# charliezhang/ringpop

Hardware: AMD Instinct MI355X
Metric: gossip rounds/sec (member-updates/s) at 65,536 sim nodes, 1/2/4/8 GPUs (higher is better)
Workload: dtype u64

## Files before the change

### include/ringpop_hip.h

```cpp
#ifndef RINGPOP_HIP_H
#define RINGPOP_HIP_H

#include <stddef.h>
#include <stdint.h>

#ifdef __cplusplus
extern "C" {
#endif

#define RP_OK 0
#define RP_ERR_INVALID (-1)
#define RP_ERR_HIP (-2)
#define RP_ERR_NOMEM (-3)
#define RP_ERR_UNSUPPORTED (-4)
#define RP_ERR_CAPACITY (-5)
#define RP_ERR_STATE (-6)

const char *rp_last_error(void);
int rp_abi_version(void);
int rp_set_device(int device);

int rp_device_malloc(size_t bytes, void **out);
int rp_device_free(void *ptr);
int rp_device_memcpy(void *dst, const void *src, size_t bytes, int kind);
// ... 54 lines not shown
typedef struct rp_sim rp_sim;
typedef struct {
    uint32_t n;
    uint32_t churn_k;
    uint64_t seed;
    uint64_t arena_entries;
    uint32_t snapshot_slots;
    uint32_t origin_slots;
    uint32_t seen_window;
    uint32_t replica_hash_shift;
    uint32_t compact_mul;
    uint32_t compact_add;
    uint32_t prefix_min;
    uint32_t ck_lane_min;
    uint32_t issue_wave;
} rp_sim_config;

typedef struct {
    uint64_t evaluated;
    uint64_t applied;
    uint64_t full_syncs;
    uint64_t messages;
    uint64_t waves;
    uint64_t pings;
    uint64_t converged;
} rp_round_stats;

int rp_sim_create(const rp_sim_config *cfg, rp_sim **out);
int rp_sim_destroy(rp_sim *sim);

// ... 158 lines not shown
```

### ringpop_amd/_lib.py

```python
import ctypes
import os

_HERE = os.path.dirname(os.path.abspath(__file__))
LIB_PATH = os.environ.get("RINGPOP_HIP_LIB") or os.path.join(_HERE, "libringpop_hip.so")

RP_OK = 0
ERRORS = {-1: "invalid argument", -2: "HIP error", -3: "out of device memory", -4: "unsupported",
          -5: "capacity exceeded", -6: "kernel error"}


class RingpopError(RuntimeError):
    def __init__(self, code, msg):
        super().__init__(f"{ERRORS.get(code, code)}: {msg}")
        self.code = code


class SimConfig(ctypes.Structure):
    _fields_ = [("n", ctypes.c_uint32), ("churn_k", ctypes.c_uint32), ("seed", ctypes.c_uint64),
                ("arena_entries", ctypes.c_uint64), ("snapshot_slots", ctypes.c_uint32),
                ("origin_slots", ctypes.c_uint32), ("seen_window", ctypes.c_uint32), ("replica_hash_shift", ctypes.c_uint32),
                ("compact_mul", ctypes.c_uint32), ("compact_add", ctypes.c_uint32), ("prefix_min", ctypes.c_uint32),
                ("ck_lane_min", ctypes.c_uint32), ("issue_wave", ctypes.c_uint32)]


class RoundStats(ctypes.Structure):
    _fields_ = [(k, ctypes.c_uint64) for k in
                ("evaluated", "applied", "full_syncs", "messages", "waves", "pings", "converged")]

    def as_dict(self):
        return {k: int(getattr(self, k)) for k, _ in self._fields_}


class RouteStats(ctypes.Structure):
    _fields_ = [(k, ctypes.c_uint64) for k in
                ("requests", "local", "delivered", "checksums_differ", "unreachable", "entry_dead", "misrouted",
                 "reserved")]

# ... 193 lines not shown
```

### ringpop_amd/build.py

```python
import json
import os
import re
import subprocess
import sys
from concurrent.futures import ThreadPoolExecutor

HERE = os.path.dirname(os.path.abspath(__file__))
CSRC = os.path.join(HERE, "csrc")
OBJ = os.path.join(HERE, "build")
LIB = os.path.join(HERE, "libringpop_hip.so")
SOURCES = ["rp_capi.hip", "rp_ring.hip", "rp_sim.hip", "rp_traffic.hip", "rp_node.hip", "rp_calib.hip"]
_INCLUDE_RE = re.compile(r'^\s*#\s*include\s+"([^"]+)"', re.M)


def included_headers(sources=SOURCES, csrc=CSRC):
    seen, todo = set(), [os.path.join(csrc, s) for s in sources]
    while todo:
        path = todo.pop()
        with open(path) as f:
            text = f.read()
        for inc in _INCLUDE_RE.findall(text):
            h = os.path.normpath(os.path.join(os.path.dirname(path), inc))
            if h not in seen and os.path.exists(h):
                seen.add(h)
                todo.append(h)
    return sorted(os.path.relpath(h, csrc) for h in seen)


HEADERS = included_headers()
ARCH = os.environ.get("RINGPOP_OFFLOAD_ARCH", "gfx950")
HIPCC = os.environ.get("HIPCC", "/opt/rocm/bin/hipcc")
FLAGS = ["-O3", "-std=c++17", "-fPIC", "--offload-arch=" + ARCH, "-Wall", "-Wno-unused-function"]
VARIANTS = {
    "diag": ["-DRP_DIAG"],
    "alt": ["-DRP_ISSUE_UNR_P1=4", "-DRP_ISSUE_UNR=4", "-DRP_ISSUE_STASH=64", "-DRP_ISSUE_P2U=1", "-DRP_SETTLED_PF=0",
            "-DRP_KPT=2", "-DRP_P2_SPLIT=1", "-DRP_CKP_SHARED=0", "-DRP_CK_SIDE=0", "-DRP_SEEN_GROUP_LOG=1",
            "-DRP_COMPACT_MUL=2u", "-DRP_COMPACT_ADD=1024u", "-DRP_LOOKUP_DIR16=0", "-DRP_RING_INCR_MAX_POINTS=0",
            "-DRP_ISSUE_WAVE=0"],
}


def _mtime(p):
    return os.path.getmtime(p) if os.path.exists(p) else 0.0


def _stamp(flags):
    return json.dumps({"hipcc": os.path.realpath(HIPCC), "arch": ARCH, "flags": flags,
                       "sources": SOURCES}, sort_keys=True)


def variant_lib(variant):
    return LIB.replace(".so", "_" + variant + ".so")

# ... 46 lines not shown
```

### ringpop_amd/csrc/rp_sim.h

```cpp
#pragma once
#include <hip/hip_runtime.h>
#include <stdint.h>

#include <string>
#include <vector>

#include "rp_common.h"

namespace rp {

enum : uint32_t {
    SIMERR_ABSENT_MEMBER = 1u << 0,
    SIMERR_TIMERS_FULL = 1u << 1,
    SIMERR_ORIGIN_FULL = 1u << 2,
    SIMERR_ARENA_FULL = 1u << 3,
    SIMERR_SNAP_FULL = 1u << 4,
    SIMERR_RINGOPS = 1u << 5,
    SIMERR_PING_FAILED = 1u << 6,
    SIMERR_PREDICATE = 1u << 7,
    SIMERR_P2_LIST = 1u << 8,
    SIMERR_LIFECYCLE = 1u << 9,
};

enum : int32_t { RESP_NONE = 0, RESP_LIST = 1, RESP_EMPTY = 2, RESP_FS_PENDING = 3, RESP_FS = 4, RESP_ERR = 5,
                 RESP_LIST_RX = 6 };

struct Resp {
    int32_t kind;
    uint32_t from;
    uint64_t off;
    uint32_t len;
    uint32_t snap;
    uint32_t ping_status;
    uint32_t plen;
    uint32_t nesc;
    uint32_t eoff;
// ... 137 lines not shown
    uint32_t* rl_len;
    uint32_t* rl_nesc;
    uint64_t* rl_inc;
    uint64_t* rl_fp;
    uint32_t* rl_csum;
    uint2* tfifo;
    uint32_t* thead;
    uint32_t* ttail;
    uint32_t tcap;
    int32_t* churn_ids;
    unsigned long long* stats;
    unsigned long long* bstats;
    uint32_t bstride;
    uint32_t* err;
    uint32_t* conv;
};

enum {
    STAT_EVALUATED = 0, STAT_APPLIED, STAT_FULLSYNC, STAT_MESSAGES, STAT_WAVES, STAT_PINGS,
    STAT_EVAL_P2, STAT_APPLIED_P2, STAT_EVAL_P3, STAT_APPLIED_P3, STAT_SCANNED_P1, STAT_EMITTED_P1,
    STAT_SCANNED_P2, STAT_EMITTED_P2, STAT_WRITTEN_P1, STAT_WRITTEN_P2,
    STAT_TOUCHED, STAT_TOUCHED_P2,
    STAT_CK_VIEWS,
    STAT_COMPACT_ISSUE, STAT_COMPACT_APPLY,
    STAT_PREFIX_PACKS,
    STAT_SAME_VIEW,
    STAT_DIAG0, STAT_DIAG1, STAT_DIAG2, STAT_DIAG3, STAT_DIAG4, STAT_DIAG5,
    STAT_WAVE_ISSUES,
    STAT_NSTATS
};

__device__ inline bool cut(const SimDev& S, uint32_t a, uint32_t b) {
    return S.part_split > 0 && S.round >= S.part_start && S.round < S.part_end &&
           ((a < S.part_split) != (b < S.part_split));
}
__host__ __device__ inline uint8_t* gossip_off(const SimDev& S) { return S.dead + S.n; }
__host__ __device__ inline uint8_t* suspicion_off(const SimDev& S) { return S.dead + 2 * (size_t)S.n; }
__device__ inline bool unreachable(const SimDev& S, uint32_t from, uint32_t to) {
    return S.dead[to] || cut(S, from, to);
}

}
```

### ringpop_amd/csrc/rp_sim.hip

```cpp
#include <hip/hip_runtime.h>

#include <algorithm>
#include <chrono>
#include <condition_variable>
#include <memory>
#include <mutex>
#include <cmath>
#include <cstdio>
#include <cstdlib>
#include <cstring>
#include <numeric>
#include <stdexcept>
#include <string>
#include <type_traits>
#include <vector>

#include "rp_block.h"
#include "rp_checksum.h"
#include "rp_common.h"
#include "rp_sim.h"
#include "rp_traffic.h"
#include "rp_whash.h"

namespace rp {
// ... 2939 lines not shown
                r.kind = RESP_EMPTY;
            } else if (!csum_known) {
                atomicOr(S.err, SIMERR_PREDICATE);
                r.kind = RESP_EMPTY;
            } else {
                uint32_t k = atomicAdd(S.snap_count, 1u);
                if (k >= S.snap_cap) { atomicOr(S.err, SIMERR_SNAP_FULL); r.kind = RESP_EMPTY; }
                else {
                    r.kind = RESP_FS_PENDING; r.snap = k;
                    S.pend_slot[k] = csum_of_sender ? (slot | PEND_SND) : slot;
                    S.pend_csum[k] = req_csum;
                }
            }
        }
        S.resp[slot] = r;
        sh.u[7] = r.kind == RESP_FS_PENDING ? r.snap : NONE;
        stat_add(S, STAT_MESSAGES, 1ull);
    }
    lds_barrier();
    if (sh.u[7] != NONE) {
        uint64_t* dst = S.snaps + (size_t)sh.u[7] * n;
        const VEnt* srow = S.view + S.row(b);
        for (uint32_t a = threadIdx.x; a < n; a += BLOCK) dst[a] = srow[a].vs;
        const uint32_t M = S.mcount[b];
        uint32_t* dord = S.snap_ord + (size_t)sh.u[7] * n;
        const uint32_t* sord = S.order + S.row(b);
        for (uint32_t i = threadIdx.x; i < M; i += BLOCK) dord[i] = sord[i];
        if (threadIdx.x == 0) S.snap_m[sh.u[7]] = M;
    }
    lds_barrier();
// ... 19 lines not shown
        const uint32_t M = S.snap_m[r.snap];
        auto src = [&](uint32_t i) {
            Change c;
            c.addr = ord[i];
            c.origin = B;
            c.vs = snap[c.addr];
            return c;
        };
        wg_apply<JOIN, PRE>(S, x, src, M, M, now, weight, phase, sh, pre);
    }
}

#ifndef RP_P2_SPLIT
#define RP_P2_SPLIT 2
#endif
constexpr uint32_t P2_SPLIT = RP_P2_SPLIT;
constexpr uint32_t P2_DEAD = 0x80000000u;
__host__ __device__ inline uint32_t p2_grid(uint32_t nl, uint32_t n, uint32_t k) {
    const uint32_t b = n / (k + 1);
    return b < nl ? (b ? b : 1u) : nl;
}
constexpr uint64_t P2_RX = 1ull << 63;
__global__ void __launch_bounds__(256) k_p2_lists(SimDev S, uint32_t* lists, uint32_t* lens, uint64_t* msgs) {
    __shared__ uint32_t wbase[P2_SPLIT + 1][4], bbase[P2_SPLIT + 1];
    const uint32_t i = blockIdx.x * blockDim.x + threadIdx.x;
    const uint32_t b = S.lo + i;
    const uint32_t c = i < S.nl ? S.g_base[b + 1] - S.g_base[b] : 0u;
    const uint64_t below = (1ull << lane_id()) - 1ull;
    const int w = threadIdx.x >> 6;
    uint64_t m[P2_SPLIT + 1];
// ... 12 lines not shown
    }
    __syncthreads();
#pragma unroll
    for (uint32_t k = 0; k <= P2_SPLIT; k++) {
        if (c > k) {
            const uint32_t e = bbase[k] + wbase[k][w] + (uint32_t)__popcll(m[k] & below);
            lists[(size_t)k * S.nl + e] = b;
            if (k < P2_SPLIT) {
                const uint32_t A = S.g_list[S.g_base[b] + k];
                lists[(size_t)(P2_SPLIT + 1 + k) * S.nl + e] = A | (S.dead[b] ? P2_DEAD : 0u);
                uint64_t* mp = msgs + ((size_t)k * S.nl + e) * 2;
                mp[0] = S.local(A) ? S.msg_off[A] : (S.rx_off[A] | P2_RX);
                mp[1] = S.msg_plen[A] | ((uint64_t)S.msg_len[A] << 32);
            }
        }
    }
}
template <bool JOIN>
__global__ void __launch_bounds__(BLOCK) __attribute__((amdgpu_waves_per_eu(RP_P3_WAVES, 8)))
k_p2_apply(SimDev S, uint64_t now, uint32_t k, const uint32_t* list, const uint32_t* len, const uint64_t* msgs) {
    RP_MERGE_SHARED(JOIN);
    const uint32_t b = __builtin_amdgcn_readfirstlane(list[blockIdx.x]);
    const uint32_t Ad = __builtin_amdgcn_readfirstlane(list[(size_t)(P2_SPLIT + 1) * S.nl + blockIdx.x]);
    const uint64_t mo = msgs[2 * blockIdx.x], ml = msgs[2 * blockIdx.x + 1];
    if (blockIdx.x >= *len) return;
    if (k == 0 && threadIdx.x == 0) note_wave(S, 1);
    const uint32_t A = Ad & ~P2_DEAD;
    if ((Ad & P2_DEAD) || cut(S, A, b)) return;
    const Change* msg = (mo & P2_RX) ? S.rxc + (mo & ~P2_RX) : S.arena + mo;
    auto src = [&](uint32_t e) { return load_msg(msg + e); };
// ... 40 lines not shown
    __shared__ Shared sh;
    uint32_t w[8];
    sload_words(rec + blockIdx.x, w);
    const uint32_t b = w[0], Ad = w[1];
    const uint64_t sv = ((uint64_t)w[3] << 32) | w[2];
    const uint64_t req_inc = ((uint64_t)w[5] << 32) | w[4], req_fp = ((uint64_t)w[7] << 32) | w[6];
    if (blockIdx.x >= *len) return;
    (void)k;
    const uint32_t A = Ad & ~(P2_DEAD | P2_NEED);
    const bool need = (Ad & P2_NEED) != 0;
    if (Ad & P2_DEAD) {
        if (threadIdx.x == 0) {
            Resp rr{};
            rr.kind = RESP_ERR; rr.from = b; rr.snap = NONE;
            S.resp[A] = rr;
            stat_add(S, STAT_MESSAGES, 1ull);
        }
        return;
    }
    respond_as_receiver<ESC, SET, SET && RP_SETTLED_PF, true>(S, b, A, req_inc, req_fp, 0u, need, A, 0, sh, sv, true);
}
template <bool ESC>
__global__ void __launch_bounds__(64) __attribute__((amdgpu_waves_per_eu(RP_WAVE_WAVES, RP_WAVE_WAVES)))
k_p2_respond_wave(SimDev S, const P2Rec* rec, const uint32_t* len) {
    __shared__ WaveShared sh;
    uint32_t w[8];
    sload_words(rec + blockIdx.x, w);
    const uint32_t b = w[0], Ad = w[1];
    const uint64_t sv = ((uint64_t)w[3] << 32) | w[2];
    const uint64_t req_inc = ((uint64_t)w[5] << 32) | w[4], req_fp = ((uint64_t)w[7] << 32) | w[6];
    if (blockIdx.x >= *len) return;
    const uint32_t A = Ad & ~(P2_DEAD | P2_NEED);
    const bool need = (Ad & P2_NEED) != 0;
    if (Ad & P2_DEAD) {
        if (threadIdx.x == 0) {
            Resp rr{};
            rr.kind = RESP_ERR; rr.from = b; rr.snap = NONE;
            S.resp[A] = rr;
            stat_add(S, STAT_MESSAGES, 1ull);
        }
        return;
    }
    const uint32_t n = S.n;
    uint64_t off;
    uint32_t pm, pe;
    const uint32_t m = wave_issue<ESC, 2>(S, b, A, req_inc, &off, sh, S.local(A) ? A : (A | DEST_REMOTE), &pm, &pe, sv);
    uint32_t snap = NONE;
    if (threadIdx.x == 0) {
        Resp r;
        r.kind = RESP_LIST; r.from = b; r.off = off; r.len = m; r.snap = NONE; r.ping_status = 0;
        r.plen = pm;
        r.nesc = pe;
        r.eoff = 0;
// ... 3 lines not shown
            } else if (!need) {
                atomicOr(S.err, SIMERR_PREDICATE);
                r.kind = RESP_EMPTY;
            } else {
                const uint32_t k = atomicAdd(S.snap_count, 1u);
                if (k >= S.snap_cap) { atomicOr(S.err, SIMERR_SNAP_FULL); r.kind = RESP_EMPTY; }
                else {
                    r.kind = RESP_FS_PENDING; r.snap = k;
                    S.pend_slot[k] = A | PEND_SND;
                    S.pend_csum[k] = 0u;
                    snap = k;
                }
            }
        }
        S.resp[A] = r;
        stat_add(S, STAT_MESSAGES, 1ull);
    }
    snap = __builtin_amdgcn_readfirstlane(snap);
    if (snap != NONE) {
        uint64_t* dst = S.snaps + (size_t)snap * n;
        const VEnt* srow = S.view + S.row(b);
        for (uint32_t a = threadIdx.x; a < n; a += 64) dst[a] = srow[a].vs;
        const uint32_t M = S.mcount[b];
        uint32_t* dord = S.snap_ord + (size_t)snap * n;
        const uint32_t* sord = S.order + S.row(b);
        for (uint32_t i = threadIdx.x; i < M; i += 64) dord[i] = sord[i];
        if (threadIdx.x == 0) S.snap_m[snap] = M;
    }
}

// ... 2 lines not shown
    __shared__ Shared sh;
    if (blockIdx.x >= *len) return;
    {
        const uint32_t b = __builtin_amdgcn_readfirstlane(list[blockIdx.x]);
        const uint32_t lo = S.g_base[b], hi = S.g_base[b + 1];
        const bool down = S.dead[b] != 0;
        uint32_t An = lo + P2_SPLIT < hi ? S.g_list[lo + P2_SPLIT] : 0u;
        for (uint32_t j = lo + P2_SPLIT; j < hi; j++) {
            const uint32_t A = __builtin_amdgcn_readfirstlane(An);
            if (j + 1 < hi) An = S.g_list[j + 1];
            if (down || cut(S, A, b)) {
                if (threadIdx.x == 0) {
                    Resp r{};
                    r.kind = RESP_ERR; r.from = b; r.snap = NONE;
                    S.resp[A] = r;
                    stat_add(S, STAT_MESSAGES, 1ull);
                }
                __syncthreads();
                continue;
            }
            const uint64_t d0 = diag_clock();
            const Change* msg = S.local(A) ? S.arena + S.msg_off[A] : S.rxc + S.rx_off[A];
            auto src = [&](uint32_t e) { return load_msg(msg + e); };
            wg_apply<JOIN>(S, b, src, S.msg_plen[A], S.msg_len[A], now, 1, 2, sh);
            const uint64_t d1 = diag_clock();
            respond_as_receiver<ESC, SET, SET && RP_SETTLED_PF>(S, b, A, S.snd_inc[A], S.snd_fp[A], 0u, S.need_csum[A] != 0, A, 0, sh, SV_NONE,
                                          true);
            if (!RP_DIAG_FINE && RP_DIAG_PHASE == 2) { DIAG_ADD(S, 3, d1 - d0); DIAG_ADD(S, 5, diag_clock() - d1); }
        }
    }
// ... 67 lines not shown
        const bool f = c < nch && flag_of(c * 64 + lane, a);
        const uint64_t m = __ballot(f);
        const uint64_t below = (1ull << lane) - 1ull;
        if (f && (uint32_t)__popcll(m & below) == p) out[j] = a;
    }
    lds_barrier();
}

template <bool JOIN, bool XS>
__global__ void __launch_bounds__(BLOCK) __attribute__((amdgpu_waves_per_eu(RP_P3_WAVES, 8))) k_phase3(SimDev S, uint64_t now,
                                                                                                    int pass) {
    RP_MERGE_SHARED(JOIN);
    const uint32_t A = S.lo + blockIdx.x;
    const int32_t T = S.target[A];
    const Resp r = S.resp[A];
    if (pass == 2 && (T < 0 || r.snap == NONE)) return;
    stage_seen(sh.seen, S.seen + S.srow(A), S.seen_words);
    ApplyPro pro;
    if (threadIdx.x == 0) pro = load_apply_pro(S, A, JOIN);
    if (T < 0 || (pass == 1 && r.snap != NONE)) return;
    if (threadIdx.x == 0) note_wave(S, 2);
    if (r.kind != RESP_ERR) apply_response<JOIN, true, XS>(S, A, r, now, 2, 3, sh, &pro);
}

template <bool ESC>
__global__ void __launch_bounds__(BLOCK) k_phase3_err(SimDev S, uint64_t now, int list_all) {
    __shared__ Shared sh;
    const uint32_t A = S.lo + blockIdx.x, n = S.n;
    if (S.target[A] < 0) return;
    if (S.resp[A].kind != RESP_ERR) return;
    if (threadIdx.x == 0) note_wave(S, 2);
    const uint32_t T = (uint32_t)S.target[A];
    __shared__ uint32_t pos[2 * 3], val[2 * 3], pick[3], sel_k;
    if (threadIdx.x == 0) {
        const uint32_t L = (uint32_t)S.npingable[A] - (is_pingable_status(v_status(S.view[S.row(A) + T].vs)) ? 1u : 0u);
        const uint32_t k = L < 3 ? L : 3;
// ... 1037 lines not shown
        const int32_t T = S.target[A];
        if (T < 0 || S.owner((uint32_t)T) != q) return false;
        const RespRec rec = rrecv[rr_idx[A]];
        v = U3{rec.psize, rec.pesc, 0};
        return true;
    }, [&](uint32_t i, const U3& p) {
        const uint32_t A = S.lo + i;
        const RespRec rec = rrecv[rr_idx[A]];
        Resp r{};
        r.from = (uint32_t)S.target[A]; r.snap = NONE; r.ping_status = 0;
        r.len = rec.len; r.plen = rec.psize; r.nesc = rec.pesc;
        r.kind = (rec.kind == RESP_LIST || rec.kind == RESP_FS) ? RESP_LIST_RX : rec.kind;
        r.off = wbase + p.a;
        r.eoff = (uint32_t)(ebase + p.b);
        S.resp[A] = r;
    });
}

__global__ void __launch_bounds__(BLOCK) k_expand_pings(SimDev S) {
    const uint32_t A = blockIdx.x;
    const int32_t T = S.target[A];
    if (S.local(A) || T < 0 || !S.local((uint32_t)T)) return;
    const uint32_t* w = S.rxw + S.rx_off[A];
    const Esc* e = S.rxe + S.rx_eoff[A];
    Change* out = S.rxc + S.rx_off[A];
    for (uint32_t i = threadIdx.x; i < S.msg_plen[A]; i += BLOCK) store_msg(out + i, wire_change(S, w[i], e));
}

struct SlotRec {
    uint32_t slot;
// ... 537 lines not shown
    DevBuf<uint64_t> xs_wabs, xs_eabs;
    DevBuf<rp::SlotRec> xsend, xrecv;
    DevBuf<unsigned long long> xsrow;
    unsigned long long* h_xsrow = nullptr;
    unsigned long long* h_xcnt = nullptr;
    unsigned long long* h_xrow = nullptr;
    uint32_t npts = 0, ncoll = 0, seen_words = 0;
    bool join_mode = false;
    bool life_mode = false;
    DevBuf<uint32_t> life_ev, tcount;
    bool fault_mode = false;
    bool issue_wave = RP_ISSUE_WAVE != 0;
    bool wave_issue_ok() const {
        return issue_wave && !fault_mode && !join_mode && n % 64 == 0 && seen_words <= rp::SEEN_STAGE_WORDS;
    }
    DevBuf<uint64_t> jvs;
    DevBuf<uint32_t> jord, jm, jcs, j_ids, j_poff, j_pidx, j_pjoin, j_seedof;
    DevBuf<int32_t> j_pseed;
    std::vector<std::string> addrs;
    uint32_t timing = 0;
    uint64_t xsent = 0;
    std::vector<TimedSpan> spans;
    std::vector<hipEvent_t> ev_pool;
    double kms[NCAT] = {0, 0, 0, 0, 0, 0, 0};
    uint64_t klaunch[NCAT] = {0, 0, 0, 0, 0, 0, 0};

    ~Shard() {
        for (auto& s : spans) { (void)hipEventDestroy(s.a); (void)hipEventDestroy(s.b); }
        for (auto e : ev_pool) (void)hipEventDestroy(e);
        if (h_xcnt) (void)hipHostFree(h_xcnt);
        if (h_xrow) (void)hipHostFree(h_xrow);
        if (h_xsrow) (void)hipHostFree(h_xsrow);
        if (xev) (void)hipEventDestroy(xev);
        for (hipEvent_t e : {ev_ck_copy, ev_ck_done, ev_merge_done, ev_pend_done})
            if (e) (void)hipEventDestroy(e);
        for (auto& sp : side_spans) { (void)hipEventDestroy(sp.a); (void)hipEventDestroy(sp.b); }
        if (st2) (void)hipStreamDestroy(st2);
        if (st && own_stream) (void)hipStreamDestroy(st);
    }
    template <class F>
    void side_timed(F&& launch) {
        if (!((timing >> 4) & 1u)) { launch(); return; }
        TimedSpan sp{4, take_event(), take_event()};
        RP_HIP(hipEventRecord(sp.a, st2));
        launch();
        RP_HIP(hipEventRecord(sp.b, st2));
        side_spans.push_back(sp);
    }

    template <class F>
    void timed(int cat, F&& launch) {
        if (!((timing >> cat) & 1u)) { launch(); return; }
// ... 38 lines not shown
                hipLaunchKernelGGL(rp::k_round_start, dim3(gx * b.n + (nl + 3) / 4), dim3(256), 0, st, b, gx, d);
            else
                hipLaunchKernelGGL(rp::k_fill_batch, dim3(gx, b.n), dim3(256), 0, st, b);
        }
        fills.clear();
    }
    hipEvent_t take_event() {
        hipEvent_t e = nullptr;
        if (!ev_pool.empty()) { e = ev_pool.back(); ev_pool.pop_back(); return e; }
        RP_HIP(hipEventCreate(&e));
        return e;
    }

    void setup();
    void group(const int32_t* dest, uint32_t nslots, bool prefilled = false, bool counted = false);
    void launch_pending(hipStream_t s) {
        hipLaunchKernelGGL(rp::k_pending, dim3(std::min(rp::grid_for(d.snap_cap, rp::NWAVE), 8192u)), dim3(rp::BLOCK), 0,
                           s, d);
    }
    void stage_start(uint32_t round, bool churn_active, uint32_t slot, const std::vector<int32_t>& dead_now,
                     bool faults, const uint32_t part[3], uint32_t storm_k);
    void stage_churn(bool churn_active, uint32_t slot, uint32_t storm_k, uint64_t now);
    void bootstrap_views(uint32_t node_lo, uint32_t count, const uint8_t* st, const uint64_t* inc,
                         const uint8_t* member_map, uint64_t seed);
    void stage_issue();
    void stage_checksums();
    void stage_ping_merge(uint64_t now);
    void stage_resp_merge(uint64_t now, bool faults);
    void stage_pr_need();
    void stage_wave(int w, uint64_t now);
// ... 72 lines not shown
        {"min_l1", d.min_l1},
        {"min_l2", d.min_l2},
        {"dangerous", d.dangerous},
        {"g_cnt", d.g_cnt},
        {"g_fill", d.g_fill},
        {"g_base", d.g_base},
        {"g_list", d.g_list},
        {"resp", d.resp},
        {"snaps", d.snaps},
        {"snap_ord", d.snap_ord},
        {"snap_m", d.snap_m},
        {"snap_count", d.snap_count},
        {"pend_slot", d.pend_slot},
        {"pend_csum", d.pend_csum},
        {"pend_done", d.pend_done},
        {"pr_n", d.pr_n},
        {"pr_errors", d.pr_errors},
        {"pr_bad", d.pr_bad},
        {"pr_done", d.pr_done},
        {"pr_inc", d.pr_inc},
        {"pr_fp", d.pr_fp},
        {"pr_csum", d.pr_csum},
        {"pr_ckv", d.pr_ckv},
        {"fdecl_bits", d.fdecl_bits},
        {"fdecl_count", d.fdecl_count},
        {"w3_dest", d.w3_dest},
        {"w4_dest", d.w4_dest},
        {"w5_dest", d.w5_dest},
        {"w6_dest", d.w6_dest},
        {"w4_err", d.w4_err},
// ... 133 lines not shown
        og_cap = 2 * nl + 64;
        og.alloc((size_t)G * (og_cap + 1));
    }
    addr_words.alloc(words.size()); addr_len.alloc(((size_t)n + 3) & ~(size_t)3);
    uint64_t acap = cfg.arena_entries ? cfg.arena_entries : std::max<uint64_t>(1ull << 22, (uint64_t)nl * 16384);
    if (acap / rp::ARENA_SHARDS >= (1ull << 32)) throw Error(RP_ERR_CAPACITY, "message arena slice above 2^32 changes");
    arena.alloc(acap); arena_cursor.alloc(16 * rp::ARENA_SHARDS);
    bstats.alloc((size_t)rp::STAT_NSTATS * n);
    RP_HIP(hipMemsetAsync(bstats.p, 0, bstats.bytes(), st));
    msg_off.alloc(n); msg_len.alloc(n); msg_plen.alloc(n); target.alloc(n); sv_word.alloc(n); snd_inc.alloc(n); snd_fp.alloc(n); snd_csum.alloc(n);
    RP_HIP(hipMemsetAsync(snd_fp.p, 0xFF, snd_fp.bytes(), st));
    g_cnt.alloc(n); g_fill.alloc(n); g_base.alloc(n + 1); g_list.alloc(3 * (size_t)n); g_tile.alloc((n + 1023) / 1024); g_bloc.alloc(n + 1);
    p2_list.alloc((size_t)(2 * rp::P2_SPLIT + 1) * nl); p2_msg.alloc((size_t)2 * rp::P2_SPLIT * nl); p2_len.alloc(rp::P2_SPLIT + 1);
    p2_rec.alloc(nl);
    resp.alloc(7 * (size_t)n);
    uint32_t scap = cfg.snapshot_slots ? cfg.snapshot_slots : std::min<uint32_t>(n, std::max<uint32_t>(4096 / G, 512));
    snaps.alloc((uint64_t)scap * n); snap_ord.alloc((uint64_t)scap * n); snap_m.alloc(scap); snap_count.alloc(1); pend_slot.alloc(scap); pend_csum.alloc(scap);
    pend_done.alloc((scap + 3u) & ~3u);
    pr_n.alloc(n); pr_errors.alloc(n); pr_bad.alloc(n); pr_done.alloc(n); pr_inc.alloc(n); pr_fp.alloc(n);
    pr_csum.alloc(n);
    const size_t n3 = 3 * (size_t)n;
    w3_dest.alloc(n3); w4_dest.alloc(n3); w5_dest.alloc(n3); w6_dest.alloc(n3); w4_err.alloc(n3);
    pq_nesc.alloc(n3); rl_nesc.alloc(n3);
    pr_ckv.alloc(n); w3cnt.alloc(n + 1); w4b.alloc(n);
    fdecl_bits.alloc((n + 31) / 32); fdecl_count.alloc(1); fdecl_all.alloc(G);
    RP_HIP(hipMemsetAsync(fdecl_bits.p, 0, fdecl_bits.bytes(), st));
    RP_HIP(hipMemsetAsync(fdecl_count.p, 0, 4, st));
    pq_off.alloc(n3); pq_len.alloc(n3); rl_off.alloc(n3); rl_len.alloc(n3); rl_inc.alloc(n3); rl_fp.alloc(n3);
    rl_csum.alloc(n3);
    const uint32_t tcap = std::min<uint32_t>(n, 16384);
// ... 79 lines not shown
    d.view = view.p; d.order = order.p; d.dko = dko.p; d.dvs = dvs.p; d.dad = dad.p; d.dhead = dhead.p; d.dtail = dtail.p;
    d.max_pb = max_pb.p; d.in_ring = in_ring.p; d.ring_count = ring_count.p; d.coll_owner = coll_owner.p;
    d.coll_of = coll_of.p; d.coll_off = coll_off.p; d.coll_ids = coll_ids.p; d.cmem_off = cmem_off.p; d.cmem = cmem.p; d.rbatch = rbatch.p; d.self_origin = self_origin.p; d.fp = fp.p; d.csum = csum.p; d.csum_valid = csum_valid.p; d.iter_index = iter_index.p;
    d.iter_round = iter_round.p; d.npingable = npingable.p; d.rng = rng.p; d.dead = dead.p;
    d.origins = origins.p; d.origin_count = origin_count.p; d.origin_cap = ocap;
    d.lorigin_count = lorigin_count.p; d.lorigin_sent = lorigin_sent.p; d.lorigin_base = lbase; d.lorigin_per = lper;
    d.alive_base = n + 1; d.alive_mask = alive_cap - 1;
    d.pq_nesc = pq_nesc.p; d.rl_nesc = rl_nesc.p; d.pr_ckv = pr_ckv.p;
    d.fdecl_bits = fdecl_bits.p; d.fdecl_count = fdecl_count.p;
    d.addr_words = addr_words.p; d.addr_len = addr_len.p;
    d.arena = arena.p; d.arena_cursor = arena_cursor.p; d.bstats = bstats.p; d.bstride = n; d.arena_cap = acap;
    d.msg_off = msg_off.p; d.msg_len = msg_len.p; d.msg_plen = msg_plen.p; d.target = target.p; d.sv_word = sv_word.p; d.snd_inc = snd_inc.p; d.snd_fp = snd_fp.p;
    d.snd_csum = snd_csum.p; d.g_cnt = g_cnt.p; d.g_fill = g_fill.p; d.g_base = g_base.p; d.g_list = g_list.p;
    d.resp = resp.p; d.snaps = snaps.p; d.snap_ord = snap_ord.p; d.snap_m = snap_m.p; d.mcount = mcount.p; d.snap_count = snap_count.p; d.snap_cap = scap; d.pend_slot = pend_slot.p;
    d.pend_csum = pend_csum.p; d.pend_done = pend_done.p;
    d.pr_n = pr_n.p; d.pr_errors = pr_errors.p; d.pr_bad = pr_bad.p; d.pr_done = pr_done.p; d.pr_inc = pr_inc.p;
    d.pr_fp = pr_fp.p; d.pr_csum = pr_csum.p; d.w3_dest = w3_dest.p; d.w4_dest = w4_dest.p; d.w5_dest = w5_dest.p;
    d.w6_dest = w6_dest.p; d.w4_err = w4_err.p; d.pq_off = pq_off.p; d.pq_len = pq_len.p; d.rl_off = rl_off.p;
    d.rl_len = rl_len.p; d.rl_inc = rl_inc.p; d.rl_fp = rl_fp.p; d.rl_csum = rl_csum.p;
    d.tfifo = tfifo.p; d.thead = thead.p; d.ttail = ttail.p; d.tcap = tcap;
    d.churn_ids = churn_ids.p; d.stats = stats.p;
    d.err = err.p; d.conv = conv.p;
    d.need_csum = need_csum.p; d.min_cnt = min_cnt.p; d.min_safe = min_safe.p; d.min_l1 = min_l1.p; d.min_l2 = min_l2.p; d.dangerous = dangerous.p; d.dlive = dlive.p; d.icount = icount.p;
    d.seen = seen.p; d.seen_words = seen_words; d.oc_snap = oc_snap.p;
    if (cfg.compact_mul || cfg.compact_add) { d.compact_mul = cfg.compact_mul; d.compact_add = cfg.compact_add; }
    else { d.compact_mul = RP_COMPACT_MUL; d.compact_add = RP_COMPACT_ADD; }
    d.prefix_min = cfg.prefix_min ? cfg.prefix_min : RP_PREFIX_MIN;
    d.ck_lane_min = cfg.ck_lane_min ? cfg.ck_lane_min : RP_CK_LANE_MIN;
    if (cfg.issue_wave) issue_wave = cfg.issue_wave == 2;
    {
        const uint32_t cap = one_per_process ? RP_SEEN_GROUP_LOG_RCCL : RP_SEEN_GROUP_LOG;
        uint32_t lg = 0;
        while (lg < cap && nl % (2u << lg) == 0) lg++;
        d.gsz_log = G > 1 ? lg : 0;
    }
    gseen.alloc(G > 1 ? (size_t)(n >> d.gsz_log) * seen_words : 1); gs_range.alloc(2);
    RP_HIP(hipMemsetAsync(gs_range.p, 0, 8, st));
    d.gseen = gseen.p; d.gs_range = gs_range.p;
    {
        uint32_t lg = 0;
        while (lg < RP_SETTLED_GROUP_LOG && nl % (2u << lg) == 0) lg++;
        d.fs_log = lg;
        const size_t pw = (n + 31) / 32;
        if (G > 1) {
// ... 167 lines not shown
    hipLaunchKernelGGL(k_group_sort, dim3(grid_for(n, 256)), dim3(256), 0, st, g_base.p, g_list.p, n);
}

void Shard::stage_start(uint32_t round, bool churn_active, uint32_t slot, const std::vector<int32_t>& dead_now,
                        bool faults, const uint32_t part[3], uint32_t storm_k) {
    using namespace rp;
    const uint64_t now = T0 + PERIOD_MS * round;
    d.round = round;
    d.part_start = part[0]; d.part_end = part[1]; d.part_split = part[2];
    fill(stats.p, stats.bytes(), 0);
    fill(arena_cursor.p, arena_cursor.bytes(), 0);
    fill(snap_count.p, 4, 0);
    fill(pend_done.p, (d.snap_cap + 3u) & ~3u, 0);
    fill(shuf_count.p, 4, 0);
    fill(p2_len.p, p2_len.bytes(), 0);
    fill(fp_mm.p, 8, 0xFF);
    fill(fp_mm.p + 1, 8, 0);
    if (faults) {
        fill(w3_dest.p, w3_dest.bytes(), 0xFF);
        fill(w4_dest.p, w4_dest.bytes(), 0xFF);
        fill(w3cnt.p, w3cnt.bytes(), 0);
        fill(w4b.p, w4b.bytes(), 0);
    }
    fill(g_cnt.p, (size_t)n * 4, 0);
    fill(g_fill.p, (size_t)n * 4, 0);
    fill(hkey.p, hkey.bytes(), 0xFF);
    fill(ck_nlead.p, 4, 0);
    fill(ck_count.p, 4, 0);
    fill_flush(true);
    if (faults) {
// ... 72 lines not shown
            const P2Rec* rk = p2_rec.p;
            if (wave_issue_ok()) {
                if (G > 1) hipLaunchKernelGGL(k_p2_respond_wave<true>, grid, dim3(64), 0, st, d, rk, p2_len.p + k);
                else hipLaunchKernelGGL(k_p2_respond_wave<false>, grid, dim3(64), 0, st, d, rk, p2_len.p + k);
            } else if (fault_mode) {
                if (G > 1) hipLaunchKernelGGL((k_p2_respond<true, true>), grid, dim3(BLOCK), 0, st, d, k, rk, p2_len.p + k);
                else hipLaunchKernelGGL((k_p2_respond<false, true>), grid, dim3(BLOCK), 0, st, d, k, rk, p2_len.p + k);
            } else {
                if (G > 1) hipLaunchKernelGGL((k_p2_respond<true, false>), grid, dim3(BLOCK), 0, st, d, k, rk, p2_len.p + k);
                else hipLaunchKernelGGL((k_p2_respond<false, false>), grid, dim3(BLOCK), 0, st, d, k, rk, p2_len.p + k);
            }
        }
        const uint32_t* lt = p2_list.p + (size_t)P2_SPLIT * nl;
        const uint32_t* nt = p2_len.p + P2_SPLIT;
        const dim3 gt(p2_grid(nl, n, P2_SPLIT));
        if (join_mode) {
            if (G > 1) hipLaunchKernelGGL((k_phase2<true, true, true>), gt, dim3(BLOCK), 0, st, d, now, lt, nt);
            else hipLaunchKernelGGL((k_phase2<false, true, true>), gt, dim3(BLOCK), 0, st, d, now, lt, nt);
        } else if (fault_mode) {
            if (G > 1) hipLaunchKernelGGL((k_phase2<true, false, true>), gt, dim3(BLOCK), 0, st, d, now, lt, nt);
            else hipLaunchKernelGGL((k_phase2<false, false, true>), gt, dim3(BLOCK), 0, st, d, now, lt, nt);
        } else {
            if (G > 1) hipLaunchKernelGGL((k_phase2<true, false, false>), gt, dim3(BLOCK), 0, st, d, now, lt, nt);
            else hipLaunchKernelGGL((k_phase2<false, false, false>), gt, dim3(BLOCK), 0, st, d, now, lt, nt);
        }
    });
    if (side_round()) {
        RP_HIP(hipEventRecord(ev_merge_done, st));
        RP_HIP(hipStreamWaitEvent(st2, ev_merge_done, 0));
        side_timed([&] {
            launch_pending(st2);
        });
        RP_HIP(hipEventRecord(ev_pend_done, st2));
    } else {
        timed(4, [&] { launch_pending(st); });
    }
}

void Shard::stage_resp_merge(uint64_t now, bool faults) {
    using namespace rp;
    timed(3, [&] {
        auto p3 = [&](int pass) {
            if (join_mode) {
                if (G > 1) hipLaunchKernelGGL((k_phase3<true, true>), dim3(nl), dim3(BLOCK), 0, st, d, now, pass);
                else hipLaunchKernelGGL((k_phase3<true, false>), dim3(nl), dim3(BLOCK), 0, st, d, now, pass);
            } else {
                if (G > 1) hipLaunchKernelGGL((k_phase3<false, true>), dim3(nl), dim3(BLOCK), 0, st, d, now, pass);
                else hipLaunchKernelGGL((k_phase3<false, false>), dim3(nl), dim3(BLOCK), 0, st, d, now, pass);
            }
        };
        if (side_round()) {
            p3(1);
            RP_HIP(hipStreamWaitEvent(st, ev_pend_done, 0));
            p3(2);
        } else {
            p3(0);
        }
        if (faults) {
            RP_HIP(hipMemsetAsync(ck_count.p, 0, 4, st));
            if (G > 1) hipLaunchKernelGGL(k_phase3_err<true>, dim3(nl), dim3(BLOCK), 0, st, d, now, 0);
            else hipLaunchKernelGGL(k_phase3_err<false>, dim3(nl), dim3(BLOCK), 0, st, d, now, 0);
            hipLaunchKernelGGL(k_pr_hist, dim3(grid_for(nl, 256)), dim3(256), 0, st, d, w3cnt.p, w4b.p,
                               faulty_unbounded ? 1u : 0u);
        }
    });
}
// ... 41 lines not shown
    timed(5, [&] {
        const uint32_t ncv = grid_for(nl, BLOCK * 4);
        if (life_mode) hipLaunchKernelGGL(k_round_end<true>, dim3(ncv + 64 * STAT_NSTATS), dim3(BLOCK), 0, st, d, fp_mm.p, ncv);
        else hipLaunchKernelGGL(k_round_end<false>, dim3(ncv + 64 * STAT_NSTATS), dim3(BLOCK), 0, st, d, fp_mm.p, ncv);
        if (G == 1)
            hipLaunchKernelGGL(k_converge_done, dim3(1), dim3(64), 0, st, d, (const unsigned long long*)fp_mm.p,
                               totals.p);
    });
    RP_HIP(hipGetLastError());
}

uint32_t Shard::read_err() {
    uint32_t e = 0;
    RP_HIP(hipMemcpyAsync(&e, err.p, 4, hipMemcpyDeviceToHost, st));
    RP_HIP(hipStreamSynchronize(st));
    if (timing) collect_timing();
    return e;
}

}


namespace rp {
struct Xfer {
    uint32_t peer;
    void* ptr;
    size_t bytes;
};
struct Xport {
    virtual ~Xport() = default;
// ... 266 lines not shown
    void run(int k_rounds, bool churn_active);
    void check_errors();
    template <class T>
    void allgather_nodes(DevBuf<T> Shard::*buf, size_t per_node);
    template <class T>
    void allgather_block(DevBuf<T> Shard::*buf, size_t per_shard);
    void allreduce_sum(DevBuf<uint32_t> Shard::*buf, size_t count);
    void alltoallv(DevBuf<Change> Shard::*sendb, DevBuf<Change> Shard::*recvb, int cat_send, int cat_recv,
                   size_t elem);
    template <class T>
    void alltoallv_t(DevBuf<T> Shard::*sendb, DevBuf<T> Shard::*recvb, int cat_send, int cat_recv);
    void read_counts();
    void origin_exchange();
    template <int W>
    void slot_exchange();
    void sync_all() { for (auto& s : sh) RP_HIP(hipStreamSynchronize(s->st)); }
    bool presized = false;
    bool loop_rank = false;
    void presize_exchange();
    hipEvent_t xdone = nullptr;
    std::vector<rp::CopyDesc> cbatch;
    void copy(void* dst, const void* src, size_t bytes) {
        if (bytes) cbatch.push_back(rp::CopyDesc{src, dst, (uint64_t)bytes});
    }
    void copy_flush() {
        for (size_t i0 = 0; i0 < cbatch.size(); i0 += rp::COPY_BATCH) {
            rp::CopyBatch b{};
            b.n = (uint32_t)std::min<size_t>(rp::COPY_BATCH, cbatch.size() - i0);
            uint64_t mx = 0;
            for (uint32_t j = 0; j < b.n; j++) { b.d[j] = cbatch[i0 + j]; mx = std::max<uint64_t>(mx, b.d[j].bytes); }
            const uint32_t gx = (uint32_t)std::min<uint64_t>(1024, std::max<uint64_t>(1, (mx + 65535) / 65536));
// ... 643 lines not shown

void rp_sim::check_errors() {
    uint32_t e = 0;
    for (auto& s : sh) e |= s->read_err();
    if (!e) return;
    std::string m = "simulation kernel error flags 0x" + std::to_string(e) + ":";
    if (e & rp::SIMERR_ABSENT_MEMBER) m += " change for an absent member (full views only);";
    if (e & rp::SIMERR_TIMERS_FULL) m += " suspicion timer FIFO full;";
    if (e & rp::SIMERR_ORIGIN_FULL) m += " origin table full;";
    if (e & rp::SIMERR_ARENA_FULL) m += " message arena full;";
    if (e & rp::SIMERR_SNAP_FULL) m += " full-sync snapshot slots exhausted;";
    if (e & rp::SIMERR_RINGOPS) m += " too many ring changes in one batch;";
    if (e & rp::SIMERR_PING_FAILED) m += " a node has no pingable member (not modelled on device);";
    if (e & rp::SIMERR_PREDICATE) m += " internal: checksum-snapshot predicate violated;";
    if (e & rp::SIMERR_P2_LIST) m += " internal: a ping-rank receiver list outgrew its launch grid;";
    if (e & rp::SIMERR_LIFECYCLE)
        m += " a leave of a node that had left, or a rejoin of a node whose own status was not leave (the join-sender"
             " is not modelled);";
    int code = (e & (rp::SIMERR_ORIGIN_FULL | rp::SIMERR_ARENA_FULL | rp::SIMERR_SNAP_FULL | rp::SIMERR_RINGOPS |
                     rp::SIMERR_TIMERS_FULL))
                   ? RP_ERR_CAPACITY
                   : (e & rp::SIMERR_LIFECYCLE) ? RP_ERR_STATE : RP_ERR_UNSUPPORTED;
    throw Error(code, m);
}


extern "C" {

static rp_sim* make_cluster(const rp_sim_config* cfg, uint32_t G, int only_rank, std::unique_ptr<rp::Xport> comm) {
    if (!cfg) throw Error(RP_ERR_INVALID, "null pointer");
// ... 1245 lines not shown
```

### ringpop_amd/sim.py

```python
import ctypes

import numpy as np

from ._lib import (RequestPending, RequestResult, RoundStats, RouteStats, SimConfig, TrafficConfig, TrafficStats, check,
                   lib, ptr)

KERNEL_CATEGORIES = ("churn", "issue", "merge_ping", "merge_resp", "checksum", "other")
STATUS_NAMES = {0: None, 1: "alive", 2: "suspect", 3: "faulty", 4: "leave"}


class Loop:

    def __init__(self, nranks):
        self._h = ctypes.c_void_p()
        self.nranks = nranks
        check(lib().rp_loop_create(nranks, ctypes.byref(self._h)))

    def close(self):
        if self._h:
            lib().rp_loop_destroy(self._h)
            self._h = ctypes.c_void_p()


class Traffic:
# ... 77 lines not shown
        return out

    def times(self):
        ms = (ctypes.c_double * 2)()
        calls = (ctypes.c_uint64 * 2)()
        peak = ctypes.c_uint64(0)
        check(lib().rp_traffic_times(self._h, ms, calls, ctypes.byref(peak)))
        return {"poll_ms": ms[0], "polls": int(calls[0]), "submit_ms": ms[1], "submits": int(calls[1]),
                "peak_pending": int(peak.value)}


class Sim:
    def __init__(self, n, seed, churn_k=None, arena_entries=0, snapshot_slots=0, origin_slots=0, failures=None,
                 partition=None, seen_window=0, replica_hash_shift=0, shards=1, rank=None, unique_id=None,
                 storm=None, addresses=None, views=None, joins=None, compact=None, loop=None, prefix_min=0, ck_lane_min=0,
                 issue_wave=0, leaves=None, rejoins=None):
        self.n = n
        self.churn_k = -(-n // 100) if churn_k is None else churn_k
        cfg = SimConfig(n=n, churn_k=self.churn_k, seed=seed, arena_entries=arena_entries,
                        snapshot_slots=snapshot_slots, origin_slots=origin_slots,
                        seen_window=seen_window, replica_hash_shift=replica_hash_shift,
                        compact_mul=compact[0] if compact else 0, compact_add=compact[1] if compact else 0,
                        prefix_min=prefix_min, ck_lane_min=ck_lane_min, issue_wave=issue_wave)
        self._h = ctypes.c_void_p()
        self._traffic = []
        self.shards = shards
        if rank is not None and loop is not None:
            check(lib().rp_sim_create_rank_loop(ctypes.byref(cfg), loop._h, rank, ctypes.byref(self._h)))
        elif rank is not None:
            uid = ctypes.create_string_buffer(bytes(unique_id), 128)
            check(lib().rp_sim_create_rank(ctypes.byref(cfg), shards, rank, uid, ctypes.byref(self._h)))
        elif shards > 1:
            check(lib().rp_sim_create_shards(ctypes.byref(cfg), shards, ctypes.byref(self._h)))
        else:
            check(lib().rp_sim_create(ctypes.byref(cfg), ctypes.byref(self._h)))
        for rnd, ids in (failures or {}).items():
            for v in ids:
                check(lib().rp_sim_fail(self._h, int(v), int(rnd)))
# ... 92 lines not shown
    def sync(self):
        check(lib().rp_sim_sync(self._h))

    def totals(self):
        st = RoundStats()
        check(lib().rp_sim_totals(self._h, ctypes.byref(st)))
        d = st.as_dict()
        d["converged_rounds"] = d.pop("converged")
        return d

    COUNTERS = ("evaluated", "applied", "full_syncs", "messages", "waves", "pings", "eval_ping_merge",
                "applied_ping_merge", "eval_resp_merge", "applied_resp_merge", "scanned_send_issue",
                "emitted_send_issue", "scanned_recv_issue", "emitted_recv_issue", "written_send_issue",
                "written_recv_issue", "touched", "touched_ping_merge", "checksum_views", "compactions_issue",
                "compactions_apply", "prefix_packs", "same_view_issues", "diag0", "diag1", "diag2", "diag3", "diag4", "diag5",
                "wave_issues")

    def counters(self):
        out = np.zeros(64, dtype=np.uint64)
        n = ctypes.c_int(0)
        check(lib().rp_sim_counters(self._h, ptr(out), 64, ctypes.byref(n)))
        d = {k: int(out[i]) for i, k in enumerate(self.COUNTERS[: n.value - 1])}
        d["converged_rounds"] = int(out[n.value - 1])
        return d

    def local_counters(self):
        out = np.zeros(64, dtype=np.uint64)
        n = ctypes.c_int(0)
        check(lib().rp_sim_local_counters(self._h, ptr(out), 64, ctypes.byref(n)))
        return {k: int(out[i]) for i, k in enumerate(self.COUNTERS[: n.value - 1])}

# ... 134 lines not shown
```

Baseline: 224.7 billion.

## Overlap early response merges with phase-2 on a side stream

Splits the phase-3 response merge into two classes. Senders whose response does not depend on the split phase-2 receiver lists and carries no pending snapshot are merged on a separate stream concurrently with phase 2, and the rest are merged afterwards. A per-slot round stamp and an error flag check that no merge reads a response before it is written. The default build leaves overlap off (RP_RESP_OVERLAP=1), so the default path always runs pass 3 then pass 4 serially, which adds a launch and extra per-node loads and stores.

Result: no change. 228.2 billion, median of 4 (+1.6%).

```diff
diff --git a/include/ringpop_hip.h b/include/ringpop_hip.h
--- a/include/ringpop_hip.h
+++ b/include/ringpop_hip.h
@@ -92,6 +92,7 @@
     uint32_t prefix_min;
     uint32_t ck_lane_min;
     uint32_t issue_wave;
+    uint32_t resp_overlap;
 } rp_sim_config;
 
 typedef struct {
diff --git a/ringpop_amd/_lib.py b/ringpop_amd/_lib.py
--- a/ringpop_amd/_lib.py
+++ b/ringpop_amd/_lib.py
@@ -20,7 +20,7 @@
                 ("arena_entries", ctypes.c_uint64), ("snapshot_slots", ctypes.c_uint32),
                 ("origin_slots", ctypes.c_uint32), ("seen_window", ctypes.c_uint32), ("replica_hash_shift", ctypes.c_uint32),
                 ("compact_mul", ctypes.c_uint32), ("compact_add", ctypes.c_uint32), ("prefix_min", ctypes.c_uint32),
-                ("ck_lane_min", ctypes.c_uint32), ("issue_wave", ctypes.c_uint32)]
+                ("ck_lane_min", ctypes.c_uint32), ("issue_wave", ctypes.c_uint32), ("resp_overlap", ctypes.c_uint32)]
 
 
 class RoundStats(ctypes.Structure):
diff --git a/ringpop_amd/build.py b/ringpop_amd/build.py
--- a/ringpop_amd/build.py
+++ b/ringpop_amd/build.py
@@ -36,7 +36,7 @@
     "alt": ["-DRP_ISSUE_UNR_P1=4", "-DRP_ISSUE_UNR=4", "-DRP_ISSUE_STASH=64", "-DRP_ISSUE_P2U=1", "-DRP_SETTLED_PF=0",
             "-DRP_KPT=2", "-DRP_P2_SPLIT=1", "-DRP_CKP_SHARED=0", "-DRP_CK_SIDE=0", "-DRP_SEEN_GROUP_LOG=1",
             "-DRP_COMPACT_MUL=2u", "-DRP_COMPACT_ADD=1024u", "-DRP_LOOKUP_DIR16=0", "-DRP_RING_INCR_MAX_POINTS=0",
-            "-DRP_ISSUE_WAVE=0"],
+            "-DRP_ISSUE_WAVE=0", "-DRP_RESP_OVERLAP=2"],
 }
 
 
diff --git a/ringpop_amd/csrc/rp_sim.h b/ringpop_amd/csrc/rp_sim.h
--- a/ringpop_amd/csrc/rp_sim.h
+++ b/ringpop_amd/csrc/rp_sim.h
@@ -20,6 +20,7 @@
     SIMERR_PREDICATE = 1u << 7,
     SIMERR_P2_LIST = 1u << 8,
     SIMERR_LIFECYCLE = 1u << 9,
+    SIMERR_RESP_ORDER = 1u << 10,
 };
 
 enum : int32_t { RESP_NONE = 0, RESP_LIST = 1, RESP_EMPTY = 2, RESP_FS_PENDING = 3, RESP_FS = 4, RESP_ERR = 5,
@@ -187,6 +188,8 @@
     uint32_t bstride;
     uint32_t* err;
     uint32_t* conv;
+    uint8_t* resp_dep;
+    uint32_t* resp_round;
 };
 
 enum {
@@ -200,6 +203,7 @@
     STAT_SAME_VIEW,
     STAT_DIAG0, STAT_DIAG1, STAT_DIAG2, STAT_DIAG3, STAT_DIAG4, STAT_DIAG5,
     STAT_WAVE_ISSUES,
+    STAT_RESP_EARLY, STAT_RESP_LATE,
     STAT_NSTATS
 };
 
diff --git a/ringpop_amd/csrc/rp_sim.hip b/ringpop_amd/csrc/rp_sim.hip
--- a/ringpop_amd/csrc/rp_sim.hip
+++ b/ringpop_amd/csrc/rp_sim.hip
@@ -2977,6 +2977,7 @@
             }
         }
         S.resp[slot] = r;
+        if (csum_of_sender) S.resp_round[slot] = S.round + 1;
         sh.u[7] = r.kind == RESP_FS_PENDING ? r.snap : NONE;
         stat_add(S, STAT_MESSAGES, 1ull);
     }
@@ -3026,6 +3027,9 @@
 #ifndef RP_P2_SPLIT
 #define RP_P2_SPLIT 2
 #endif
+#ifndef RP_RESP_OVERLAP
+#define RP_RESP_OVERLAP 1
+#endif
 constexpr uint32_t P2_SPLIT = RP_P2_SPLIT;
 constexpr uint32_t P2_DEAD = 0x80000000u;
 __host__ __device__ inline uint32_t p2_grid(uint32_t nl, uint32_t n, uint32_t k) {
@@ -3068,6 +3072,11 @@
                 mp[1] = S.msg_plen[A] | ((uint64_t)S.msg_len[A] << 32);
             }
         }
+    }
+    if (c > P2_SPLIT) {
+        S.resp_dep[b] = 1;
+        const uint32_t g0 = S.g_base[b];
+        for (uint32_t j = P2_SPLIT; j < c; j++) S.resp_dep[S.g_list[g0 + j]] = 1;
     }
 }
 template <bool JOIN>
@@ -3138,6 +3147,7 @@
             Resp rr{};
             rr.kind = RESP_ERR; rr.from = b; rr.snap = NONE;
             S.resp[A] = rr;
+            S.resp_round[A] = S.round + 1;
             stat_add(S, STAT_MESSAGES, 1ull);
         }
         return;
@@ -3161,6 +3171,7 @@
             Resp rr{};
             rr.kind = RESP_ERR; rr.from = b; rr.snap = NONE;
             S.resp[A] = rr;
+            S.resp_round[A] = S.round + 1;
             stat_add(S, STAT_MESSAGES, 1ull);
         }
         return;
@@ -3194,6 +3205,7 @@
             }
         }
         S.resp[A] = r;
+        S.resp_round[A] = S.round + 1;
         stat_add(S, STAT_MESSAGES, 1ull);
     }
     snap = __builtin_amdgcn_readfirstlane(snap);
@@ -3226,6 +3238,7 @@
                     Resp r{};
                     r.kind = RESP_ERR; r.from = b; r.snap = NONE;
                     S.resp[A] = r;
+                    S.resp_round[A] = S.round + 1;
                     stat_add(S, STAT_MESSAGES, 1ull);
                 }
                 __syncthreads();
@@ -3323,12 +3336,20 @@
     const uint32_t A = S.lo + blockIdx.x;
     const int32_t T = S.target[A];
     const Resp r = S.resp[A];
+    const uint32_t dep = S.resp_dep[A], rr = S.resp_round[A];
     if (pass == 2 && (T < 0 || r.snap == NONE)) return;
+    const bool early = dep == 0 && r.snap == NONE;
+    if (pass == 3 && (dep != 0 || T < 0 || !early)) return;
+    if (pass == 4 && (T < 0 || early)) return;
     stage_seen(sh.seen, S.seen + S.srow(A), S.seen_words);
     ApplyPro pro;
     if (threadIdx.x == 0) pro = load_apply_pro(S, A, JOIN);
     if (T < 0 || (pass == 1 && r.snap != NONE)) return;
-    if (threadIdx.x == 0) note_wave(S, 2);
+    if (threadIdx.x == 0) {
+        note_wave(S, 2);
+        if (rr != S.round + 1) atomicOr(S.err, SIMERR_RESP_ORDER);
+        if (pass >= 3 && r.kind != RESP_ERR) stat_add(S, pass == 3 ? STAT_RESP_EARLY : STAT_RESP_LATE, 1ull);
+    }
     if (r.kind != RESP_ERR) apply_response<JOIN, true, XS>(S, A, r, now, 2, 3, sh, &pro);
 }
 
@@ -4396,6 +4417,7 @@
         r.off = wbase + p.a;
         r.eoff = (uint32_t)(ebase + p.b);
         S.resp[A] = r;
+        S.resp_round[A] = S.round + 1;
     });
 }
 
@@ -4963,6 +4985,14 @@
     bool wave_issue_ok() const {
         return issue_wave && !fault_mode && !join_mode && n % 64 == 0 && seen_words <= rp::SEEN_STAGE_WORDS;
     }
+    bool resp_overlap = RP_RESP_OVERLAP == 2;
+    DevBuf<uint8_t> resp_dep;
+    DevBuf<uint32_t> resp_round;
+    hipStream_t st_resp = nullptr;
+    hipEvent_t ev_resp_ready = nullptr, ev_early_done = nullptr;
+    bool early_in_flight = false;
+    bool resp_two_class() const { return G == 1 && !fault_mode && !join_mode; }
+    bool resp_overlap_round() const { return resp_two_class() && resp_overlap && st_resp && !((timing >> 3) & 1u); }
     DevBuf<uint64_t> jvs;
     DevBuf<uint32_t> jord, jm, jcs, j_ids, j_poff, j_pidx, j_pjoin, j_seedof;
     DevBuf<int32_t> j_pseed;
@@ -4985,6 +5015,9 @@
             if (e) (void)hipEventDestroy(e);
         for (auto& sp : side_spans) { (void)hipEventDestroy(sp.a); (void)hipEventDestroy(sp.b); }
         if (st2) (void)hipStreamDestroy(st2);
+        for (hipEvent_t e : {ev_resp_ready, ev_early_done})
+            if (e) (void)hipEventDestroy(e);
+        if (st_resp) (void)hipStreamDestroy(st_resp);
         if (st && own_stream) (void)hipStreamDestroy(st);
     }
     template <class F>
@@ -5053,6 +5086,16 @@
 
     void setup();
     void group(const int32_t* dest, uint32_t nslots, bool prefilled = false, bool counted = false);
+    void launch_p3(hipStream_t s, uint64_t now, int pass) {
+        using namespace rp;
+        if (join_mode) {
+            if (G > 1) hipLaunchKernelGGL((k_phase3<true, true>), dim3(nl), dim3(BLOCK), 0, s, d, now, pass);
+            else hipLaunchKernelGGL((k_phase3<true, false>), dim3(nl), dim3(BLOCK), 0, s, d, now, pass);
+        } else {
+            if (G > 1) hipLaunchKernelGGL((k_phase3<false, true>), dim3(nl), dim3(BLOCK), 0, s, d, now, pass);
+            else hipLaunchKernelGGL((k_phase3<false, false>), dim3(nl), dim3(BLOCK), 0, s, d, now, pass);
+        }
+    }
     void launch_pending(hipStream_t s) {
         hipLaunchKernelGGL(rp::k_pending, dim3(std::min(rp::grid_for(d.snap_cap, rp::NWAVE), 8192u)), dim3(rp::BLOCK), 0,
                            s, d);
@@ -5155,6 +5198,8 @@
         {"pend_slot", d.pend_slot},
         {"pend_csum", d.pend_csum},
         {"pend_done", d.pend_done},
+        {"resp_dep", d.resp_dep},
+        {"resp_round", d.resp_round},
         {"pr_n", d.pr_n},
         {"pr_errors", d.pr_errors},
         {"pr_bad", d.pr_bad},
@@ -5318,6 +5363,9 @@
     p2_list.alloc((size_t)(2 * rp::P2_SPLIT + 1) * nl); p2_msg.alloc((size_t)2 * rp::P2_SPLIT * nl); p2_len.alloc(rp::P2_SPLIT + 1);
     p2_rec.alloc(nl);
     resp.alloc(7 * (size_t)n);
+    resp_dep.alloc(((size_t)n + 3) & ~(size_t)3);
+    resp_round.alloc(n);
+    RP_HIP(hipMemsetAsync(resp_round.p, 0, resp_round.bytes(), st));
     uint32_t scap = cfg.snapshot_slots ? cfg.snapshot_slots : std::min<uint32_t>(n, std::max<uint32_t>(4096 / G, 512));
     snaps.alloc((uint64_t)scap * n); snap_ord.alloc((uint64_t)scap * n); snap_m.alloc(scap); snap_count.alloc(1); pend_slot.alloc(scap); pend_csum.alloc(scap);
     pend_done.alloc((scap + 3u) & ~3u);
@@ -5427,6 +5475,7 @@
     d.snd_csum = snd_csum.p; d.g_cnt = g_cnt.p; d.g_fill = g_fill.p; d.g_base = g_base.p; d.g_list = g_list.p;
     d.resp = resp.p; d.snaps = snaps.p; d.snap_ord = snap_ord.p; d.snap_m = snap_m.p; d.mcount = mcount.p; d.snap_count = snap_count.p; d.snap_cap = scap; d.pend_slot = pend_slot.p;
     d.pend_csum = pend_csum.p; d.pend_done = pend_done.p;
+    d.resp_dep = resp_dep.p; d.resp_round = resp_round.p;
     d.pr_n = pr_n.p; d.pr_errors = pr_errors.p; d.pr_bad = pr_bad.p; d.pr_done = pr_done.p; d.pr_inc = pr_inc.p;
     d.pr_fp = pr_fp.p; d.pr_csum = pr_csum.p; d.w3_dest = w3_dest.p; d.w4_dest = w4_dest.p; d.w5_dest = w5_dest.p;
     d.w6_dest = w6_dest.p; d.w4_err = w4_err.p; d.pq_off = pq_off.p; d.pq_len = pq_len.p; d.rl_off = rl_off.p;
@@ -5441,6 +5490,11 @@
     d.prefix_min = cfg.prefix_min ? cfg.prefix_min : RP_PREFIX_MIN;
     d.ck_lane_min = cfg.ck_lane_min ? cfg.ck_lane_min : RP_CK_LANE_MIN;
     if (cfg.issue_wave) issue_wave = cfg.issue_wave == 2;
+    if (cfg.resp_overlap) resp_overlap = cfg.resp_overlap == 2;
+    if (G == 1) {
+        RP_HIP(hipStreamCreateWithFlags(&st_resp, hipStreamNonBlocking));
+        for (hipEvent_t* e : {&ev_resp_ready, &ev_early_done}) RP_HIP(hipEventCreateWithFlags(e, hipEventDisableTiming));
+    }
     {
         const uint32_t cap = one_per_process ? RP_SEEN_GROUP_LOG_RCCL : RP_SEEN_GROUP_LOG;
         uint32_t lg = 0;
@@ -5638,6 +5692,7 @@
     fill(pend_done.p, (d.snap_cap + 3u) & ~3u, 0);
     fill(shuf_count.p, 4, 0);
     fill(p2_len.p, p2_len.bytes(), 0);
+    fill(resp_dep.p, resp_dep.bytes(), 0);
     fill(fp_mm.p, 8, 0xFF);
     fill(fp_mm.p + 1, 8, 0);
     if (faults) {
@@ -5740,6 +5795,8 @@
         const uint32_t* lt = p2_list.p + (size_t)P2_SPLIT * nl;
         const uint32_t* nt = p2_len.p + P2_SPLIT;
         const dim3 gt(p2_grid(nl, n, P2_SPLIT));
+        early_in_flight = resp_overlap_round();
+        if (early_in_flight) RP_HIP(hipEventRecord(ev_resp_ready, st));
         if (join_mode) {
             if (G > 1) hipLaunchKernelGGL((k_phase2<true, true, true>), gt, dim3(BLOCK), 0, st, d, now, lt, nt);
             else hipLaunchKernelGGL((k_phase2<false, true, true>), gt, dim3(BLOCK), 0, st, d, now, lt, nt);
@@ -5749,6 +5806,11 @@
         } else {
             if (G > 1) hipLaunchKernelGGL((k_phase2<true, false, false>), gt, dim3(BLOCK), 0, st, d, now, lt, nt);
             else hipLaunchKernelGGL((k_phase2<false, false, false>), gt, dim3(BLOCK), 0, st, d, now, lt, nt);
+        }
+        if (early_in_flight) {
+            RP_HIP(hipStreamWaitEvent(st_resp, ev_resp_ready, 0));
+            launch_p3(st_resp, now, 3);
+            RP_HIP(hipEventRecord(ev_early_done, st_resp));
         }
     });
     if (side_round()) {
@@ -5766,16 +5828,13 @@
 void Shard::stage_resp_merge(uint64_t now, bool faults) {
     using namespace rp;
     timed(3, [&] {
-        auto p3 = [&](int pass) {
-            if (join_mode) {
-                if (G > 1) hipLaunchKernelGGL((k_phase3<true, true>), dim3(nl), dim3(BLOCK), 0, st, d, now, pass);
-                else hipLaunchKernelGGL((k_phase3<true, false>), dim3(nl), dim3(BLOCK), 0, st, d, now, pass);
-            } else {
-                if (G > 1) hipLaunchKernelGGL((k_phase3<false, true>), dim3(nl), dim3(BLOCK), 0, st, d, now, pass);
-                else hipLaunchKernelGGL((k_phase3<false, false>), dim3(nl), dim3(BLOCK), 0, st, d, now, pass);
-            }
-        };
-        if (side_round()) {
+        auto p3 = [&](int pass) { launch_p3(st, now, pass); };
+        if (resp_two_class()) {
+            if (early_in_flight) RP_HIP(hipStreamWaitEvent(st, ev_early_done, 0));
+            else p3(3);
+            early_in_flight = false;
+            p3(4);
+        } else if (side_round()) {
             p3(1);
             RP_HIP(hipStreamWaitEvent(st, ev_pend_done, 0));
             p3(2);
@@ -5847,6 +5906,7 @@
     uint32_t e = 0;
     RP_HIP(hipMemcpyAsync(&e, err.p, 4, hipMemcpyDeviceToHost, st));
     RP_HIP(hipStreamSynchronize(st));
+    if (st_resp) RP_HIP(hipStreamSynchronize(st_resp));
     if (timing) collect_timing();
     return e;
 }
@@ -6143,7 +6203,12 @@
     void origin_exchange();
     template <int W>
     void slot_exchange();
-    void sync_all() { for (auto& s : sh) RP_HIP(hipStreamSynchronize(s->st)); }
+    void sync_all() {
+        for (auto& s : sh) {
+            RP_HIP(hipStreamSynchronize(s->st));
+            if (s->st_resp) RP_HIP(hipStreamSynchronize(s->st_resp));
+        }
+    }
     bool presized = false;
     bool loop_rank = false;
     void presize_exchange();
@@ -6817,6 +6882,7 @@
     if (e & rp::SIMERR_PING_FAILED) m += " a node has no pingable member (not modelled on device);";
     if (e & rp::SIMERR_PREDICATE) m += " internal: checksum-snapshot predicate violated;";
     if (e & rp::SIMERR_P2_LIST) m += " internal: a ping-rank receiver list outgrew its launch grid;";
+    if (e & rp::SIMERR_RESP_ORDER) m += " internal: a sender's response merge ran before this round's response was written;";
     if (e & rp::SIMERR_LIFECYCLE)
         m += " a leave of a node that had left, or a rejoin of a node whose own status was not leave (the join-sender"
              " is not modelled);";
diff --git a/ringpop_amd/sim.py b/ringpop_amd/sim.py
--- a/ringpop_amd/sim.py
+++ b/ringpop_amd/sim.py
@@ -115,14 +115,15 @@
     def __init__(self, n, seed, churn_k=None, arena_entries=0, snapshot_slots=0, origin_slots=0, failures=None,
                  partition=None, seen_window=0, replica_hash_shift=0, shards=1, rank=None, unique_id=None,
                  storm=None, addresses=None, views=None, joins=None, compact=None, loop=None, prefix_min=0, ck_lane_min=0,
-                 issue_wave=0, leaves=None, rejoins=None):
+                 issue_wave=0, leaves=None, rejoins=None, resp_overlap=0):
         self.n = n
         self.churn_k = -(-n // 100) if churn_k is None else churn_k
         cfg = SimConfig(n=n, churn_k=self.churn_k, seed=seed, arena_entries=arena_entries,
                         snapshot_slots=snapshot_slots, origin_slots=origin_slots,
                         seen_window=seen_window, replica_hash_shift=replica_hash_shift,
                         compact_mul=compact[0] if compact else 0, compact_add=compact[1] if compact else 0,
-                        prefix_min=prefix_min, ck_lane_min=ck_lane_min, issue_wave=issue_wave)
+                        prefix_min=prefix_min, ck_lane_min=ck_lane_min, issue_wave=issue_wave,
+                        resp_overlap=resp_overlap)
         self._h = ctypes.c_void_p()
         self._traffic = []
         self.shards = shards
@@ -245,7 +246,7 @@
                 "emitted_send_issue", "scanned_recv_issue", "emitted_recv_issue", "written_send_issue",
                 "written_recv_issue", "touched", "touched_ping_merge", "checksum_views", "compactions_issue",
                 "compactions_apply", "prefix_packs", "same_view_issues", "diag0", "diag1", "diag2", "diag3", "diag4", "diag5",
-                "wave_issues")
+                "wave_issues", "resp_early", "resp_late")
 
     def counters(self):
         out = np.zeros(64, dtype=np.uint64)
```
